# acg-team/ProGraphMSA

Hardware: AMD Instinct MI355X
Metric: DP cell-updates/sec (GCUPS) + wall-clock on 256 seqs × 1000 aa, WAG (higher is better)
Workload: dtype f32

## Files before the change

include/pgm_hip.h:

```cpp
#ifndef PGM_HIP_H_
#define PGM_HIP_H_

#include <stdint.h>
#include <stddef.h>

#ifdef __cplusplus
extern "C" {
#endif

#define PGM_OK 0
#define PGM_ERR_INVALID 1
#define PGM_ERR_DEVICE 2
#define PGM_ERR_BACKTRACK 3
#define PGM_ERR_NOMEM 4

#define PGM_GAP 0xFFFFFFFFu


typedef struct pgm_graph {
    uint32_t n;
    uint32_t dim;
    const double *sites;
    const int32_t *e_rowptr;
    const uint32_t *e_col;
// ... 23 lines not shown
} pgm_align_out;

typedef struct pgm_ctx pgm_ctx;
typedef struct pgm_align_batch pgm_align_batch;

int pgm_device_count(void);
int pgm_ctx_create(int device, pgm_ctx **out);
void pgm_ctx_destroy(pgm_ctx *ctx);
const char *pgm_last_error(void);
int pgm_ctx_device_info(pgm_ctx *ctx, char *name, size_t name_len, int *cu_count);

int pgm_align_graphs_batch(pgm_ctx *ctx, uint32_t njobs, const pgm_graph *const *g1,
                           const pgm_graph *const *g2, const pgm_model *const *model,
                           const pgm_scores *scores, pgm_align_out *out);

int pgm_align_batch_create(pgm_ctx *ctx, uint32_t njobs, const pgm_graph *const *g1,
                           const pgm_graph *const *g2, const pgm_model *const *model,
                           const pgm_scores *scores, pgm_align_batch **out);
#define PGM_BATCH_KEEP_MATRICES 1u
int pgm_align_batch_create_ex(pgm_ctx *ctx, uint32_t njobs, const pgm_graph *const *g1,
                              const pgm_graph *const *g2, const pgm_model *const *model,
                              const pgm_scores *scores, uint32_t flags, pgm_align_batch **out);
typedef struct pgm_site_ref {
    const double *dev_sites;
    const uint32_t *node_map;
    uint32_t ncols;
} pgm_site_ref;
int pgm_align_batch_create_res(pgm_ctx *ctx, uint32_t njobs, const pgm_graph *const *g1,
                               const pgm_graph *const *g2, const pgm_model *const *model,
                               const pgm_scores *scores, uint32_t flags, const pgm_site_ref *res1,
                               const pgm_site_ref *res2, pgm_align_batch **out);
int pgm_align_graphs_batch_res(pgm_ctx *ctx, uint32_t njobs, const pgm_graph *const *g1,
                               const pgm_graph *const *g2, const pgm_model *const *model,
                               const pgm_scores *scores, const pgm_site_ref *res1,
                               const pgm_site_ref *res2, pgm_align_out *out);
int pgm_align_batch_run(pgm_ctx *ctx, pgm_align_batch *b);
int pgm_align_batch_fetch(pgm_ctx *ctx, pgm_align_batch *b, pgm_align_out *out);
void pgm_align_batch_destroy(pgm_ctx *ctx, pgm_align_batch *b);
uint64_t pgm_align_batch_cells(const pgm_align_batch *b);
int pgm_align_batch_time(pgm_ctx *ctx, pgm_align_batch *b, int reps, float *ms_prep,
                         float *ms_emission, float *ms_fill, float *ms_traceback);
int pgm_align_batch_stage_times(pgm_align_batch *b, int reset, float *ms_prep, float *ms_emission, float *ms_fill,
                                uint32_t *launches);
int pgm_align_batch_job_times(pgm_ctx *ctx, pgm_align_batch *b, uint64_t *ticks);
int pgm_align_batch_test_stall(pgm_align_batch *b, uint32_t job, uint32_t band, uint32_t spin_limit);
int pgm_test_cu_shares(uint32_t cus, double lean_cost, uint32_t nlean, double band_cost, uint32_t nbands, double rest_cost,
                       uint32_t nrest, uint32_t ncrit, double longest_chain, uint32_t *out4);
#define PGM_PLAN_HEAD 23
#define PGM_PLAN_DHEAD 9
#define PGM_PLAN_JOB 19
int pgm_test_batch_plan(uint32_t njobs, const pgm_graph *const *g1, const pgm_graph *const *g2, const pgm_model *const *model,
                        const pgm_scores *scores, uint32_t flags, const pgm_site_ref *res1, const pgm_site_ref *res2, uint32_t cus,
                        uint32_t *head, double *dhead, uint32_t *job_fields, uint32_t *items, uint32_t *bands, uint32_t *lean_list, int32_t *tblist);
int pgm_align_batch_read_matrices(pgm_ctx *ctx, pgm_align_batch *b, uint32_t job, float *M,
                                  float *X, float *Y, float *W, float *S);

int pgm_nw_pairs_batch(pgm_ctx *ctx, uint32_t dim, const int32_t *score, int32_t gap_open,
                       int32_t gap_extend, uint32_t nseq, const int8_t *syms,
                       const uint32_t *offs, uint32_t npairs, const uint32_t *pi,
                       const uint32_t *pj, int32_t *counts, uint32_t *gaps);
#define PGM_NW_REDUCED 1u
int pgm_nw_pairs_submit(pgm_ctx *ctx, uint32_t dim, const int32_t *score, int32_t gap_open,
                        int32_t gap_extend, uint32_t nseq, const int8_t *syms,
                        const uint32_t *offs, uint32_t npairs, const uint32_t *pi,
                        const uint32_t *pj, uint32_t flags, int32_t *counts, uint32_t *gaps, int *ticket);
int pgm_nw_pairs_wait(pgm_ctx *ctx, int ticket);
float pgm_nw_last_kernel_ms(pgm_ctx *ctx);
void *pgm_host_alloc(size_t bytes);
void pgm_host_free(void *p);

int pgm_csprofile_load(pgm_ctx *ctx, uint32_t K, uint32_t ncols, const double *lprofiles,
                       const double *centre, const double *priors);
int pgm_csprofile_create_batch(pgm_ctx *ctx, uint32_t nseq, const int8_t *syms,
                               const uint32_t *offs, const double *tau, const double *pi,
                               const double *p_uniform, double *out, const uint64_t *out_offs);
int pgm_csprofile_create_batch_res(pgm_ctx *ctx, uint32_t nseq, const int8_t *syms,
                                   const uint32_t *offs, const double *tau, const double *pi,
                                   const double *p_uniform, const double **dev);
float pgm_csprofile_last_kernel_ms(pgm_ctx *ctx);

typedef struct pgm_mldist_model {
    uint32_t dim;
    const double *Q, *V, *Vi, *sigma;
    double dist_max, var_max, var_min, cutoff_dist, min_dist, max_dist, indel_rate;
    int32_t mldist, mldist_gap;
} pgm_mldist_model;
int pgm_mldist_batch(pgm_ctx *ctx, const pgm_mldist_model *model, uint32_t npairs, const int32_t *counts,
                     const uint32_t *gaps, const double *seqlen, double *dist, double *var);

int pgm_prealigned_counts_batch(pgm_ctx *ctx, uint32_t dim, uint32_t nrows, uint32_t ncols, const int8_t *rows,
                                uint32_t npairs, const uint32_t *pi, const uint32_t *pj, int32_t *counts,
                                uint32_t *gaps);
int pgm_kmer_cosine(pgm_ctx *ctx, uint32_t nseq, uint32_t ncols, const int32_t *counts, double *cosine);
int pgm_kmer_cosine_multi(pgm_ctx *ctx, uint32_t nfam, const uint32_t *nseq, uint32_t ncols, const int32_t *counts, double *cosine);
int pgm_prealigned_counts_multi(pgm_ctx *ctx, uint32_t dim, uint32_t nfam, const uint32_t *nrows, const uint32_t *ncols,
                                const int8_t *rows, uint32_t npairs, const uint32_t *fam, const uint32_t *pi, const uint32_t *pj,
                                int32_t *counts, uint32_t *gaps);
int pgm_prealigned_counts_resampled(pgm_ctx *ctx, uint32_t dim, uint32_t nrows, uint32_t ncols, const int8_t *rows, uint32_t nrep,
                                    const uint32_t *cols, uint32_t npairs, const uint32_t *pi, const uint32_t *pj, int32_t *counts,
                                    uint32_t *gaps);
float pgm_dist_last_kernel_ms(pgm_ctx *ctx);

typedef struct pgm_merge_job {
    uint32_t dim, n1, n2, nnodes;
    const double *sites1, *sites2;
    const double *P1, *P2;
// ... 129 lines not shown
```

prographmsa_amd/__init__.py:

```python
import ctypes as C
import os

_HERE = os.path.dirname(os.path.abspath(__file__))
LIB_PATH = os.path.join(_HERE, "lib", "libpgm_hip.so")
PGMSA_PATH = os.path.join(_HERE, "bin", "pgmsa")

PGM_OK, PGM_ERR_INVALID, PGM_ERR_DEVICE, PGM_ERR_BACKTRACK, PGM_ERR_NOMEM = 0, 1, 2, 3, 4
PGM_GAP = 0xFFFFFFFF
PGM_BATCH_KEEP_MATRICES = 1
PGM_NW_REDUCED = 1
PGM_MERGE_RESIDENT = 1


class pgm_graph(C.Structure):
    _fields_ = [("n", C.c_uint32), ("dim", C.c_uint32), ("sites", C.POINTER(C.c_double)),
                ("e_rowptr", C.POINTER(C.c_int32)), ("e_col", C.POINTER(C.c_uint32)), ("e_val", C.POINTER(C.c_float)),
                ("r_rowptr", C.POINTER(C.c_int32)), ("r_col", C.POINTER(C.c_uint32)), ("r_units", C.POINTER(C.c_uint32))]


class pgm_model(C.Structure):
    _fields_ = [("M", C.POINTER(C.c_double)), ("pi", C.POINTER(C.c_double))]


class pgm_scores(C.Structure):
    _fields_ = [(n, C.c_float) for n in ("gap_init", "gap_extend", "match_init", "end_match", "end_gap", "end_skip",
                                         "start_gap", "start_init", "repeat_init", "repeat_ext")]


class pgm_mldist_model(C.Structure):
    _fields_ = [("dim", C.c_uint32), ("Q", C.POINTER(C.c_double)), ("V", C.POINTER(C.c_double)), ("Vi", C.POINTER(C.c_double)),
                ("sigma", C.POINTER(C.c_double))] + [(n, C.c_double) for n in ("dist_max", "var_max", "var_min", "cutoff_dist", "min_dist", "max_dist", "indel_rate")] \
        + [("mldist", C.c_int32), ("mldist_gap", C.c_int32)]


class pgm_merge_job(C.Structure):
    _fields_ = [("dim", C.c_uint32), ("n1", C.c_uint32), ("n2", C.c_uint32), ("nnodes", C.c_uint32),
                ("sites1", C.POINTER(C.c_double)), ("sites2", C.POINTER(C.c_double)), ("P1", C.POINTER(C.c_double)), ("P2", C.POINTER(C.c_double)),
                ("k1", C.POINTER(C.c_uint32)), ("k2", C.POINTER(C.c_uint32)), ("g2_with_P1", C.POINTER(C.c_uint8)), ("profiles", C.POINTER(C.c_double))]


class pgm_site_ref(C.Structure):
    _fields_ = [("dev_sites", C.POINTER(C.c_double)), ("node_map", C.POINTER(C.c_uint32)), ("ncols", C.c_uint32)]


class pgm_gapmask_job(C.Structure):
    _fields_ = [("src", C.POINTER(C.c_uint64)), ("mapping", C.POINTER(C.c_uint32)), ("dst", C.POINTER(C.c_uint64)),
                ("nrows", C.c_uint32), ("ncols_in", C.c_uint32), ("ncols_out", C.c_uint32)]


class pgm_parsimony_job(C.Structure):
    _fields_ = [("masks", C.POINTER(C.c_uint64)), ("children", C.POINTER(C.c_uint32)), ("nleaves", C.c_uint32), ("ncols", C.c_uint32)]


class pgm_wls_job(C.Structure):
    _fields_ = [("label", C.POINTER(C.c_int8)), ("offset", C.POINTER(C.c_double)), ("nsub", C.c_uint32)]


class pgm_bionj_join(C.Structure):
    _fields_ = [("index1", C.c_uint32), ("index2", C.c_uint32), ("dist1", C.c_double), ("dist2", C.c_double)]


class pgm_bionj_pair(C.Structure):
    _fields_ = [("index1", C.c_uint32), ("index2", C.c_uint32)]


class pgm_align_out(C.Structure):
    _fields_ = [("score", C.c_float), ("n_tr_indels", C.c_uint32), ("len", C.c_uint32), ("status", C.c_int32),
                ("map1", C.POINTER(C.c_uint32)), ("map2", C.POINTER(C.c_uint32))]


EXPORTS = [
    "pgm_device_count", "pgm_ctx_create", "pgm_ctx_destroy", "pgm_last_error", "pgm_ctx_device_info",
    "pgm_align_graphs_batch", "pgm_align_batch_create", "pgm_align_batch_create_ex", "pgm_align_batch_create_res", "pgm_align_graphs_batch_res", "pgm_align_batch_run", "pgm_align_batch_fetch",
    "pgm_align_batch_destroy", "pgm_align_batch_cells", "pgm_align_batch_test_stall", "pgm_test_cu_shares", "pgm_test_batch_plan", "pgm_align_batch_stage_times", "pgm_align_batch_job_times", "pgm_align_batch_time", "pgm_align_batch_read_matrices",
    "pgm_nw_pairs_batch", "pgm_nw_pairs_submit", "pgm_nw_pairs_wait", "pgm_nw_last_kernel_ms", "pgm_host_alloc", "pgm_host_free", "pgm_csprofile_load", "pgm_csprofile_create_batch", "pgm_csprofile_create_batch_res",
    "pgm_csprofile_last_kernel_ms", "pgm_mldist_batch", "pgm_prealigned_counts_batch", "pgm_kmer_cosine", "pgm_dist_last_kernel_ms",
    "pgm_kmer_cosine_multi", "pgm_prealigned_counts_multi", "pgm_prealigned_counts_resampled",
    "pgm_merge_profiles_batch", "pgm_merge_profiles_batch_ex", "pgm_resident_reset", "pgm_resident_onehot", "pgm_resident_import", "pgm_merge_last_kernel_ms",
    "pgm_gapmask_extend_batch", "pgm_gap_parsimony_batch", "pgm_parsimony_last_kernel_ms",
    "pgm_wls_load", "pgm_wls_pair_sums_batch", "pgm_wls_last_kernel_ms", "pgm_wls_last_launches",
    "pgm_bionj", "pgm_bionj_multi", "pgm_bionj_last_launches", "pgm_bionj_last_kernel_ms",
    "pgm_bionj_plan", "pgm_bionj_plan_multi",
    "pgm_msa_agreement", "pgm_agreement_last_kernel_ms",
    "pgm_transfer_min", "pgm_transfer_last_kernel_ms", "pgm_transfer_taxa",
    "pgm_tree_likelihood", "pgm_treelik_last_kernel_ms", "pgm_tree_likelihood_rates", "pgm_tree_ancestral", "pgm_tree_nni", "pgm_tree_nni_edge", "pgm_tree_spr",
    "pgm_tree_ancestral_joint", "pgm_tree_ancestral_sample",
    "pgm_resampled_sums", "pgm_resample_last_kernel_ms",
]


def _load():
    if not os.path.exists(LIB_PATH):
        raise ImportError("libpgm_hip.so is not built (%s); run `python -c 'import __graft_entry__ as g; g.build()'` "
                          "— there is no CPU fallback for the hot path" % LIB_PATH)
    lib = C.CDLL(LIB_PATH)
    vp, u32, i32 = C.c_void_p, C.c_uint32, C.c_int32
    PG, PM = C.POINTER(C.POINTER(pgm_graph)), C.POINTER(C.POINTER(pgm_model))
    sig = {
        "pgm_device_count": (C.c_int, []),
        "pgm_ctx_create": (C.c_int, [C.c_int, C.POINTER(vp)]),
        "pgm_ctx_destroy": (None, [vp]),
        "pgm_last_error": (C.c_char_p, []),
        "pgm_ctx_device_info": (C.c_int, [vp, C.c_char_p, C.c_size_t, C.POINTER(C.c_int)]),
        "pgm_align_graphs_batch": (C.c_int, [vp, u32, PG, PG, PM, C.POINTER(pgm_scores), C.POINTER(pgm_align_out)]),
        "pgm_align_batch_create": (C.c_int, [vp, u32, PG, PG, PM, C.POINTER(pgm_scores), C.POINTER(vp)]),
        "pgm_align_batch_create_ex": (C.c_int, [vp, u32, PG, PG, PM, C.POINTER(pgm_scores), u32, C.POINTER(vp)]),
        "pgm_align_batch_create_res": (C.c_int, [vp, u32, PG, PG, PM, C.POINTER(pgm_scores), u32, C.POINTER(pgm_site_ref), C.POINTER(pgm_site_ref), C.POINTER(vp)]),
        "pgm_align_graphs_batch_res": (C.c_int, [vp, u32, PG, PG, PM, C.POINTER(pgm_scores), C.POINTER(pgm_site_ref), C.POINTER(pgm_site_ref), C.POINTER(pgm_align_out)]),
        "pgm_align_batch_run": (C.c_int, [vp, vp]),
        "pgm_align_batch_fetch": (C.c_int, [vp, vp, C.POINTER(pgm_align_out)]),
        "pgm_align_batch_destroy": (None, [vp, vp]),
        "pgm_align_batch_cells": (C.c_uint64, [vp]),
        "pgm_align_batch_test_stall": (C.c_int, [vp, u32, u32, u32]),
        "pgm_test_cu_shares": (C.c_int, [u32, C.c_double, u32, C.c_double, u32, C.c_double, u32, u32, C.c_double, C.POINTER(C.c_uint32)]),
        "pgm_test_batch_plan": (C.c_int, [u32, PG, PG, PM, C.POINTER(pgm_scores), u32, C.POINTER(pgm_site_ref), C.POINTER(pgm_site_ref), u32,
                                          C.POINTER(u32), C.POINTER(C.c_double)] + [C.POINTER(u32)] * 4 + [C.POINTER(i32)]),
        "pgm_align_batch_stage_times": (C.c_int, [vp, C.c_int] + [C.POINTER(C.c_float)] * 3 + [C.POINTER(u32)]),
        "pgm_align_batch_job_times": (C.c_int, [vp, vp, C.POINTER(C.c_uint64)]),
        "pgm_align_batch_time": (C.c_int, [vp, vp, C.c_int] + [C.POINTER(C.c_float)] * 4),
        "pgm_align_batch_read_matrices": (C.c_int, [vp, vp, u32] + [C.POINTER(C.c_float)] * 5),
        "pgm_nw_pairs_batch": (C.c_int, [vp, u32, C.POINTER(i32), i32, i32, u32, C.POINTER(C.c_int8), C.POINTER(u32), u32,
                                         C.POINTER(u32), C.POINTER(u32), C.POINTER(i32), C.POINTER(u32)]),
        "pgm_nw_pairs_submit": (C.c_int, [vp, u32, C.POINTER(i32), i32, i32, u32, C.POINTER(C.c_int8), C.POINTER(u32), u32,
                                          C.POINTER(u32), C.POINTER(u32), u32, C.POINTER(i32), C.POINTER(u32), C.POINTER(C.c_int)]),
        "pgm_nw_pairs_wait": (C.c_int, [vp, C.c_int]),
        "pgm_host_alloc": (vp, [C.c_size_t]),
        "pgm_host_free": (None, [vp]),
        "pgm_nw_last_kernel_ms": (C.c_float, [vp]),
        "pgm_csprofile_load": (C.c_int, [vp, u32, u32] + [C.POINTER(C.c_double)] * 3),
        "pgm_csprofile_create_batch": (C.c_int, [vp, u32, C.POINTER(C.c_int8), C.POINTER(u32)] + [C.POINTER(C.c_double)] * 4
                                       + [C.POINTER(C.c_uint64)]),
        "pgm_csprofile_create_batch_res": (C.c_int, [vp, u32, C.POINTER(C.c_int8), C.POINTER(u32)] + [C.POINTER(C.c_double)] * 3
                                           + [C.POINTER(C.POINTER(C.c_double))]),
        "pgm_csprofile_last_kernel_ms": (C.c_float, [vp]),
        "pgm_mldist_batch": (C.c_int, [vp, C.POINTER(pgm_mldist_model), u32, C.POINTER(i32), C.POINTER(u32)] + [C.POINTER(C.c_double)] * 3),
        "pgm_prealigned_counts_batch": (C.c_int, [vp, u32, u32, u32, C.POINTER(C.c_int8), u32, C.POINTER(u32), C.POINTER(u32), C.POINTER(i32), C.POINTER(u32)]),
        "pgm_kmer_cosine": (C.c_int, [vp, u32, u32, C.POINTER(i32), C.POINTER(C.c_double)]),
        "pgm_dist_last_kernel_ms": (C.c_float, [vp]),
        "pgm_kmer_cosine_multi": (C.c_int, [vp, u32, C.POINTER(u32), u32, C.POINTER(i32), C.POINTER(C.c_double)]),
        "pgm_prealigned_counts_multi": (C.c_int, [vp, u32, u32, C.POINTER(u32), C.POINTER(u32), C.POINTER(C.c_int8), u32, C.POINTER(u32), C.POINTER(u32),
                                                  C.POINTER(u32), C.POINTER(i32), C.POINTER(u32)]),
        "pgm_prealigned_counts_resampled": (C.c_int, [vp, u32, u32, u32, C.POINTER(C.c_int8), u32, C.POINTER(u32), u32, C.POINTER(u32), C.POINTER(u32),
                                                      C.POINTER(i32), C.POINTER(u32)]),
        "pgm_merge_profiles_batch": (C.c_int, [vp, u32, C.POINTER(pgm_merge_job)]),
        "pgm_merge_profiles_batch_ex": (C.c_int, [vp, u32, C.POINTER(pgm_merge_job), u32, C.POINTER(C.POINTER(C.c_double))]),
        "pgm_resident_reset": (C.c_int, [vp]),
        "pgm_resident_onehot": (C.c_int, [vp, u32, u32, C.POINTER(C.c_int8), C.POINTER(u32), C.POINTER(C.POINTER(C.c_double))]),
        "pgm_resident_import": (C.c_int, [vp, vp, C.POINTER(C.c_double), C.c_uint64, C.POINTER(C.POINTER(C.c_double))]),
        "pgm_merge_last_kernel_ms": (C.c_float, [vp]),
        "pgm_gapmask_extend_batch": (C.c_int, [vp, u32, C.POINTER(pgm_gapmask_job)]),
        "pgm_gap_parsimony_batch": (C.c_int, [vp, u32, C.POINTER(pgm_parsimony_job), C.POINTER(u32)]),
        "pgm_parsimony_last_kernel_ms": (C.c_float, [vp]),
        "pgm_wls_load": (C.c_int, [vp, u32, C.POINTER(C.c_double), C.POINTER(C.c_double)]),
        "pgm_wls_pair_sums_batch": (C.c_int, [vp, u32, C.POINTER(pgm_wls_job), C.POINTER(C.c_double)]),
        "pgm_wls_last_kernel_ms": (C.c_float, [vp]),
        "pgm_wls_last_launches": (C.c_uint32, [vp]),
        "pgm_bionj": (C.c_int, [vp, u32, C.POINTER(C.c_double), C.POINTER(C.c_double), C.POINTER(pgm_bionj_join), C.POINTER(C.c_double)]),
        "pgm_bionj_multi": (C.c_int, [vp, u32, C.POINTER(u32), C.POINTER(C.c_double), C.POINTER(C.c_double), C.POINTER(pgm_bionj_join), C.POINTER(C.c_double)]),
        "pgm_bionj_last_launches": (C.c_uint32, [vp]),
        "pgm_bionj_last_kernel_ms": (C.c_float, [vp]),
        "pgm_bionj_plan": (C.c_int, [vp, u32, C.POINTER(C.c_double), C.POINTER(C.c_double), C.POINTER(pgm_bionj_pair), C.POINTER(pgm_bionj_join), C.POINTER(C.c_double)]),
        "pgm_bionj_plan_multi": (C.c_int, [vp, u32, C.POINTER(u32), C.POINTER(C.c_double), C.POINTER(C.c_double), C.POINTER(pgm_bionj_pair), C.POINTER(pgm_bionj_join), C.POINTER(C.c_double)]),
        "pgm_msa_agreement": (C.c_int, [vp, u32, u32, u32, C.POINTER(i32), C.POINTER(u32), C.POINTER(u32)]),
        "pgm_agreement_last_kernel_ms": (C.c_float, [vp]),
        "pgm_transfer_min": (C.c_int, [vp, u32, u32, C.POINTER(C.c_uint64), u32, C.POINTER(u32), C.POINTER(C.c_uint64), C.POINTER(u32)]),
        "pgm_transfer_last_kernel_ms": (C.c_float, [vp]),
        "pgm_transfer_taxa": (C.c_int, [vp, u32, u32, C.POINTER(C.c_uint64), C.POINTER(u32), u32, C.POINTER(u32), C.POINTER(C.c_uint64),
                                        C.POINTER(u32), C.POINTER(u32), C.POINTER(u32), C.POINTER(u32)]),
        "pgm_tree_likelihood": (C.c_int, [vp, u32, u32, u32, C.POINTER(u32), u32, C.POINTER(C.c_int8), C.POINTER(C.c_double), C.POINTER(C.c_double), C.c_int,
                                          C.POINTER(C.c_double), C.POINTER(i32), C.POINTER(C.c_double), C.POINTER(C.c_double)]),
        "pgm_treelik_last_kernel_ms": (C.c_float, [vp]),
        "pgm_tree_likelihood_rates": (C.c_int, [vp, u32, u32, u32, C.POINTER(u32), u32, C.POINTER(C.c_int8), C.POINTER(C.c_double), u32, C.POINTER(C.c_double),
                                                C.POINTER(C.c_double), C.c_int, C.POINTER(C.c_double), C.POINTER(i32), C.POINTER(C.c_double), C.POINTER(C.c_double),
# ... 317 lines not shown
```

prographmsa_amd/csrc/pgm_align_kernels.h:

```cpp
#ifndef PGM_ALIGN_KERNELS_H_
#define PGM_ALIGN_KERNELS_H_

#include <hip/hip_runtime.h>
#include <math.h>
#include <type_traits>
#include "pgm_device.h"

#define PGM_NEG_INF (-INFINITY)

__device__ __forceinline__ float pgm_ls_log_add(float x, float add) {
    const float a = 2.44247459618085927548717403238913328776812604856113966238617812902399112761292613763080658235564f;
    const float b = -4.2040783745848554315883301529007786406310628696382695994938550046831869207082846248658671f;
    const float c = -0.72123729809042963774358701619456664388406302428056983119308906451199556380646306f;
    const uint32_t bits = __float_as_uint(x);
    const float e = (float)((int32_t)(bits >> 23) - 126);
    const float d = __uint_as_float(((bits << 9) >> 9) ^ 0x3f000000u);
    float t = __fdiv_rn(b, __fsub_rn(d, c));
    const float u = __fadd_rn(e, a);
    t = __fadd_rn(t, add);
    t = __fadd_rn(t, u);
    return t;
}

__device__ __forceinline__ float pgm_emission_finish(float num, float ay, float bx, float match_init) {
    float q = __fdiv_rn(num, __fmul_rn(ay, bx));
    if (q != q) q = __uint_as_float(0xFFC00000u);
    return pgm_ls_log_add(q, match_init);
}

template <int DMAX, int NODES>
__global__ void __launch_bounds__(NODES) pgm_prep_kernel(const PgmJob *__restrict__ jobs, int *__restrict__ sync, uint32_t sync_ints) {
    extern __shared__ float prep_lds[];
    {
        const uint32_t nthreads = gridDim.x * gridDim.y * gridDim.z * NODES;
        const uint32_t gid = ((blockIdx.z * gridDim.y + blockIdx.y) * gridDim.x + blockIdx.x) * NODES + threadIdx.x;
        for (uint32_t i = gid; i < sync_ints; i += nthreads) sync[i] = 0;
    }
    const PgmJob &J = jobs[blockIdx.x];
    const bool first = blockIdx.y == 0;
    const uint32_t n = first ? J.n1 : J.n2;
    const uint32_t v0 = blockIdx.z * NODES;
    if (v0 >= n) return;
    if (J.tabhdr && J.tabhdr[0] == 0) {
        const uint32_t nc = J.dim + 2u;
        bool any = n - 1u >= v0 && n - 1u < v0 + (uint32_t)NODES;
        for (uint32_t c = 0; c < nc; ++c) {
            const uint32_t r = (uint32_t)J.tabhdr[1u + (first ? 0u : nc) + c];
            any = any || (r != 0u && r - 1u >= v0 && r - 1u < v0 + (uint32_t)NODES);
        }
        if (!any) return;
    }
    const uint32_t D = J.dim, DP = J.dp, ST = D + 1;
    float *Mf = prep_lds;
    float *pif = prep_lds + D * D;
    float *nl = pif + D;
    const uint32_t nn = min((uint32_t)NODES, n - v0);
    {
        const int32_t *pp = first ? J.pp1 : J.pp2;
        const uint32_t *pc = first ? J.pc1 : J.pc2, *pu = first ? J.pu1 : J.pu2;
        const float *pv = first ? J.pv1 : J.pv2;
        PgmTbNode *rec = (first ? J.tb1 : J.tb2) + v0;
        for (uint32_t i = threadIdx.x; i < nn * PGM_TB_PK; i += NODES) {
            const uint32_t node = i / PGM_TB_PK, k = i % PGM_TB_PK;
            const int32_t eb = pp[v0 + node];
            const uint32_t cnt = (uint32_t)(pp[v0 + node + 1] - eb);
            const int32_t e = cnt == 0u ? 0 : eb + (int32_t)min(k, cnt - 1u);
            if (k == 0) rec[node].cnt = cnt;
            rec[node].c[k] = pc[e]; rec[node].v[k] = pv[e]; rec[node].u[k] = pu[e];
        }
    }
    if (!first) for (uint32_t i = threadIdx.x; i < D * D; i += NODES) Mf[i] = (float)J.M[i];
    for (uint32_t i = threadIdx.x; i < D; i += NODES) pif[i] = (float)J.pi[i];
    const double *sites = first ? J.sites1 : J.sites2;
    const uint32_t *smap = first ? J.smap1 : J.smap2;
    float *dst = (first ? J.g1f : J.t2) + (size_t)DP * v0;
    for (uint32_t i = threadIdx.x; i < nn * D; i += NODES) {
        const uint32_t node = v0 + i / D;
        const float g = (float)sites[(size_t)D * (smap ? smap[node] : node) + i % D];
        nl[(i / D) * ST + (i % D)] = g;
        if (first && DP == D) dst[i] = g;
// ... 44 lines not shown
        const uint32_t node = i / DP, k = i % DP;
        dst[i] = k < D ? nl[node * ST + k] : 0.0f;
    }
}

#define PGM_TAB_HDR 136
__global__ void __launch_bounds__(256) pgm_classify_kernel(const PgmJob *__restrict__ jobs) {
    const PgmJob &J = jobs[blockIdx.x];
    if (!J.tabhdr) return;
    const bool first = blockIdx.y == 0;
    const uint32_t n = first ? J.n1 : J.n2, D = J.dim;
    const double *sites = first ? J.sites1 : J.sites2;
    const uint32_t *smap = first ? J.smap1 : J.smap2;
    uint8_t *cls = (uint8_t *)(first ? J.cls1 : J.cls2);
    const float uni = (float)(1.0 / (double)D);
    for (uint32_t v = blockIdx.z * blockDim.x + threadIdx.x; v < n; v += gridDim.z * blockDim.x) {
        const double *col = sites + (size_t)D * (smap ? smap[v] : v);
        uint32_t nz = 0, sym = 0;
        bool same = true;
        float vs = 0.f;
        const float g0 = (float)col[0];
        for (uint32_t k = 0; k < D; ++k) {
            const float g = (float)col[k];
            if (g != 0.0f) { ++nz; sym = k; vs = g; }
            same = same && g == g0;
        }
        uint32_t c = 255u;
        if (nz == 0u) c = D + 1u;
        else if (nz == 1u && vs == 1.0f) c = sym;
        else if (same && g0 == uni) c = D;
        cls[v] = (uint8_t)c;
        if (c == 255u) atomicOr(J.tabhdr, 1);
        else atomicCAS(J.tabhdr + 1 + (first ? 0u : D + 2u) + c, 0, (int)v + 1);
    }
}

__device__ __forceinline__ size_t pgm_cell_index(const PgmJob &J, uint32_t y, uint32_t x) {
    const uint32_t b = y / PGM_ROWS, l = PGM_HALO + (y - b * PGM_ROWS);
    return ((size_t)b * J.tsteps + (x + l)) * 64u + l;
}
__device__ __forceinline__ float4 pgm_load_cell(const PgmJob &J, uint32_t y, uint32_t x) {
    return J.cells[pgm_cell_index(J, y, x)];
}

__device__ __forceinline__ float pgm_dpp_wave_shr1(float src, float lane0_value) {
    return __int_as_float(__builtin_amdgcn_update_dpp(__float_as_int(lane0_value), __float_as_int(src), 0x138, 0xf, 0xf, false));
}

#define PGM_GLOBAL __attribute__((address_space(1)))
typedef float pgm_v4f __attribute__((ext_vector_type(4)));
template <class T> __device__ __forceinline__ T pgm_gld(const T *p) { return *(const PGM_GLOBAL T *)(uintptr_t)p; }
#define PGM_EM_TB 4
template <int DP, int RB>
__global__ void __launch_bounds__(4 * PGM_ROWS) pgm_emission_skew_kernel(const PgmJob *__restrict__ jobs) {
    typedef float pgm_v2f __attribute__((ext_vector_type(2)));
    constexpr int NT = DP / 4;
    constexpr int COLS = 64 + PGM_EM_TB * PGM_BLOCK - PGM_HALO - 1;
    constexpr int STR = DP + 1;
    __shared__ pgm_v2f tp[(COLS + 1) * STR];
    __shared__ float bq[COLS];
    const PgmJob &J = jobs[blockIdx.z];
    const uint32_t tb0 = blockIdx.x * PGM_EM_TB;
    const uint32_t rsh = J.rshift, nvb = J.nb << rsh;
    if (tb0 >= J.nblk || 4u * RB * blockIdx.y >= nvb) return;
    if (J.tabhdr && pgm_gld(J.tabhdr) == 0) return;
    auto row_of = [&](uint32_t v, uint32_t lane_) { return ((((v >> rsh) << 6) + lane_) << rsh) | (v & ((1u << rsh) - 1u)); };
    auto sblock_of = [&](uint32_t v, uint32_t tb_) { return ((((size_t)(v >> rsh) * J.nblk + tb_) << rsh) | (v & ((1u << rsh) - 1u))); };
    const uint32_t t0 = tb0 * PGM_BLOCK;
    const int cbase = (int)t0 - 63;
    if ((DP == 20 || DP == 4) && RB == 1) {
        constexpr int TE = DP + 1;
        float *const tab = (float *)tp;
        static_assert(COLS * TE <= (COLS + 1) * STR * 2, "score table must fit the column staging area");
        static_assert(DP > 20 || TE <= 32, "row classes must fit As");
        __shared__ float As[32];
        const uint32_t fb0 = 4u * blockIdx.y + threadIdx.x / PGM_ROWS;
        const uint32_t fl = threadIdx.x % PGM_ROWS;
        const bool active = fb0 < nvb;
        int sym = DP;
        bool plain = true;
        float a_row = 0.f;
        if (active) {
            const uint32_t y = row_of(fb0, fl);
            const uint32_t yc = (y + 1 < J.n1) ? y : 0u;
            const float4 *src = (const float4 *)(J.g1f + (size_t)DP * yc);
            int nz = 0;
#pragma unroll
            for (int q = 0; q < NT; ++q) {
                const float4 v = src[q];
                const float vv[4] = {v.x, v.y, v.z, v.w};
#pragma unroll
                for (int u = 0; u < 4; ++u)
                    if (vv[u] != 0.0f) { ++nz; sym = 4 * q + u; plain = plain && vv[u] == 1.0f; }
            }
            plain = plain && nz <= 1;
            a_row = J.a1[yc];
        }
        if (threadIdx.x < 32) As[threadIdx.x] = 0.f;
        if (__syncthreads_and(plain ? 1 : 0)) {
            if (active) As[sym] = a_row;
            __syncthreads();
            const float mi = J.sc.match_init;
            constexpr int NE = (COLS * TE + 4 * PGM_ROWS - 1) / (4 * PGM_ROWS);
            float tt[NE], tb2[NE];
#pragma unroll
            for (int e = 0; e < NE; ++e) {
                const int i = (int)threadIdx.x + e * 4 * PGM_ROWS;
// ... 17 lines not shown
                if (tb >= J.nblk) break;
                float out[PGM_BLOCK];
#pragma unroll
                for (int i = 0; i < PGM_BLOCK; ++i) out[i] = tab[((int)(tb * PGM_BLOCK) + i - l - cbase) * TE + sym];
                PGM_GLOBAL pgm_v4f *dst = Sq + (sblock_of(fb0, tb) * 64u + (uint32_t)l) * (PGM_BLOCK / 4);
#pragma unroll
                for (int q = 0; q < PGM_BLOCK / 4; ++q) dst[q] = pgm_v4f{out[4 * q], out[4 * q + 1], out[4 * q + 2], out[4 * q + 3]};
            }
            return;
        }
    }
    const float4 *t2q = (const float4 *)J.t2;
    float *tpf = (float *)tp;
    for (int i = threadIdx.x; i < (COLS + 1) * NT; i += 4 * PGM_ROWS) {
        const int ci = i / NT, q = i % NT, c = cbase + ci;
        float4 v = make_float4(0.f, 0.f, 0.f, 0.f);
        if (c >= 0 && c <= (int)J.ncol) v = t2q[(size_t)NT * c + q];
        const float vv[4] = {v.x, v.y, v.z, v.w};
#pragma unroll
        for (int u = 0; u < 4; ++u) {
            const int k = 4 * q + u;
            if (ci < COLS) tpf[2 * (ci * STR + k)] = vv[u];
            if (ci > 0) tpf[2 * ((ci - 1) * STR + k) + 1] = vv[u];
        }
    }
    for (int i = threadIdx.x; i < COLS; i += 4 * PGM_ROWS) {
        const int col = cbase + i;
        bq[i] = (col >= 0 && col <= (int)J.ncol) ? J.b2[col] : 0.f;
    }
    __syncthreads();
    const uint32_t b0 = (4u * blockIdx.y + threadIdx.x / PGM_ROWS) * RB;
    const int l = PGM_HALO + (int)(threadIdx.x % PGM_ROWS);
    if (b0 >= nvb) return;
    float gy[RB][DP], ay[RB];
#pragma unroll
    for (int r = 0; r < RB; ++r) {
        const uint32_t y = row_of(b0 + (uint32_t)r, (uint32_t)(l - PGM_HALO));
        const uint32_t yc = (y + 1 < J.n1) ? y : 0u;
        const float4 *src = (const float4 *)(J.g1f + (size_t)DP * yc);
#pragma unroll
        for (int q = 0; q < NT; ++q) {
            const float4 v = src[q];
            gy[r][4 * q] = v.x; gy[r][4 * q + 1] = v.y; gy[r][4 * q + 2] = v.z; gy[r][4 * q + 3] = v.w;
        }
        ay[r] = J.a1[yc];
    }
    const float mi = J.sc.match_init;
    const uint32_t nblk = J.nblk;
    PGM_GLOBAL pgm_v4f *const Sq = (PGM_GLOBAL pgm_v4f *)(uintptr_t)J.S;
#pragma unroll 1
    for (int w = 0; w < PGM_EM_TB; ++w) {
        const uint32_t tb = tb0 + w;
        if (tb >= nblk) break;
        float out[RB][PGM_BLOCK];
#pragma unroll
        for (int i = 0; i < PGM_BLOCK; i += 2) {
            const int ci = (int)(tb * PGM_BLOCK) + i - l - cbase;
            const pgm_v2f *tc = tp + ci * STR;
            pgm_v2f acc[RB];
#pragma unroll
            for (int r = 0; r < RB; ++r) acc[r] = pgm_v2f{0.0f, 0.0f};
#pragma unroll
            for (int k = 0; k < DP; ++k) {
                const pgm_v2f tk = tc[k];
#pragma unroll
                for (int r = 0; r < RB; ++r) {
                    const pgm_v2f g = {gy[r][k], gy[r][k]};
                    acc[r] = acc[r] + g * tk;
                }
            }
#pragma unroll
            for (int r = 0; r < RB; ++r) {
                out[r][i] = pgm_emission_finish(acc[r].x, ay[r], bq[ci], mi);
                out[r][i + 1] = pgm_emission_finish(acc[r].y, ay[r], bq[ci + 1], mi);
            }
        }
#pragma unroll
        for (int r = 0; r < RB; ++r) {
            if (b0 + (uint32_t)r < nvb) {
                PGM_GLOBAL pgm_v4f *dst = Sq + (sblock_of(b0 + (uint32_t)r, tb) * 64u + (uint32_t)l) * (PGM_BLOCK / 4);
#pragma unroll
                for (int q = 0; q < PGM_BLOCK / 4; ++q) dst[q] = pgm_v4f{out[r][4 * q], out[r][4 * q + 1], out[r][4 * q + 2], out[r][4 * q + 3]};
            }
        }
    }
}

__device__ __forceinline__ int pgm_wave_max8(uint32_t v) {
    int m = __builtin_amdgcn_ballot_w64(v >= 8u) != 0 ? 8 : 0;
    m += __builtin_amdgcn_ballot_w64(v >= (uint32_t)(m + 4)) != 0 ? 4 : 0;
    m += __builtin_amdgcn_ballot_w64(v >= (uint32_t)(m + 2)) != 0 ? 2 : 0;
    m += __builtin_amdgcn_ballot_w64(v >= (uint32_t)(m + 1)) != 0 ? 1 : 0;
    return m;
}

__device__ __forceinline__ __amdgpu_buffer_rsrc_t pgm_band_rsrc(float4 *base, uint32_t bytes) {
    const uint64_t p = (uint64_t)base;
    const uint32_t lo = __builtin_amdgcn_readfirstlane((uint32_t)p), hi = __builtin_amdgcn_readfirstlane((uint32_t)(p >> 32));
    return __builtin_amdgcn_make_buffer_rsrc((void *)(((uint64_t)hi << 32) | lo), 0, __builtin_amdgcn_readfirstlane(bytes), 0x00020000);
}
__device__ __forceinline__ void pgm_store_cell_masked(__amdgpu_buffer_rsrc_t rsrc, uint32_t t, int lane, bool on, float Mv, float Xv, float Wv, float Yv) {
    typedef uint32_t pgm_v4u __attribute__((ext_vector_type(4)));
    pgm_v4u v;
    v.x = __float_as_uint(Mv); v.y = __float_as_uint(Xv); v.z = __float_as_uint(Wv); v.w = __float_as_uint(Yv);
    __builtin_amdgcn_raw_buffer_store_b128(v, rsrc, (on ? (uint32_t)lane * 16u : 0x80000000u) + t * 1024u, 0, 16);
}
__device__ __forceinline__ float4 pgm_gload4(const float4 *p) {
    const pgm_v4f v = *(const PGM_GLOBAL pgm_v4f *)(uintptr_t)p;
    return make_float4(v.x, v.y, v.z, v.w);
}
__device__ __forceinline__ float2 pgm_gload_cell_wy(const float4 *p) {
    const unsigned long long v = __hip_atomic_load((const PGM_GLOBAL unsigned long long *)(uintptr_t)p + 1, __ATOMIC_RELAXED, __HIP_MEMORY_SCOPE_AGENT);
    return make_float2(__uint_as_float((uint32_t)v), __uint_as_float((uint32_t)(v >> 32)));
}
__device__ __forceinline__ float2 pgm_load_cell_mx(const float4 *p) {
    const unsigned long long v = __hip_atomic_load((const PGM_GLOBAL unsigned long long *)(uintptr_t)p, __ATOMIC_RELAXED, __HIP_MEMORY_SCOPE_AGENT);
    return make_float2(__uint_as_float((uint32_t)v), __uint_as_float((uint32_t)(v >> 32)));
}
__device__ __forceinline__ float2 pgm_load_cell_wy(const float4 *p) {
    const unsigned long long v = __hip_atomic_load((const PGM_GLOBAL unsigned long long *)(uintptr_t)p + 1, __ATOMIC_RELAXED, __HIP_MEMORY_SCOPE_AGENT);
    return make_float2(__uint_as_float((uint32_t)v), __uint_as_float((uint32_t)(v >> 32)));
}

struct PgmPred {
    const int32_t *pp; const uint32_t *pc; const float *pv; const uint32_t *pu;
};
__device__ __forceinline__ float pgm_mark_value(const PgmPred &P, int32_t e) {
    const uint32_t u = P.pu[e];
    if (u == 0) return P.pv[e];
    const uint32_t units = u & 0x7fffffffu;
    if (units == 0) return INFINITY;
    return __fadd_rn(INFINITY, __fmul_rn(INFINITY, (float)(units - 1)));
}

struct PgmMapOut {
// ... 2212 lines not shown
```

prographmsa_amd/csrc/pgm_capi.hip:

```cpp
#include <hip/hip_runtime.h>

#include <algorithm>
#include <cmath>
#include <cstdio>
#include <thread>
#include <atomic>
#include <chrono>
#include <queue>
#include <cstdlib>
#include <cstring>
#include <numeric>
#include <optional>
#include <mutex>
#include <string>
#include <unordered_set>
#include <vector>
#include <sys/mman.h>

#include "pgm_align_kernels.h"
#include "pgm_crit_kernels.h"
#include "pgm_nw_kernels.h"
#include "pgm_csprofile_kernels.h"
#include "pgm_dist_kernels.h"
#include "pgm_merge_kernels.h"
// ... 820 lines not shown
        if (res.status != PGM_OK) rc = res.status;
        if (copied[i]) continue;
        out[i].score = res.score;
        out[i].n_tr_indels = res.n_tr_indels;
        out[i].len = res.len;
        out[i].status = res.status;
        if (res.status != PGM_OK) rc = res.status;
        if (!out[i].map1 || !out[i].map2) return fail(PGM_ERR_INVALID, "null mapping buffer");
        if (res.len > b->jobs[i].n1 + b->jobs[i].n2) return fail(PGM_ERR_DEVICE, "corrupt result length");
        memcpy(out[i].map1, b->h_out + b->map1_off[i], 4 * (size_t)res.len);
        memcpy(out[i].map2, b->h_out + b->map2_off[i], 4 * (size_t)res.len);
    }
    if (rc != PGM_OK) g_err = "backtracking failed";
    return rc;
}

void pgm_align_batch_destroy(pgm_ctx *ctx, pgm_align_batch *b) {
    if (!b) return;
    if (ctx) { (void)hipSetDevice(ctx->device); (void)hipStreamSynchronize(ctx->stream); }
    if (ctx && ctx->stream2) (void)hipStreamSynchronize(ctx->stream2);
    if (ctx && ctx->stream3) (void)hipStreamSynchronize(ctx->stream3);
    if (ctx && ctx->stream4) (void)hipStreamSynchronize(ctx->stream4);
    for (int k = 0; k < 5; ++k)
        if (b->ev[k]) (void)hipEventDestroy(b->ev[k]);
    if (b->ev_fork) (void)hipEventDestroy(b->ev_fork);
    if (b->ev_join) (void)hipEventDestroy(b->ev_join);
    if (b->ev_join_b) (void)hipEventDestroy(b->ev_join_b);
    if (b->ev_join_c) (void)hipEventDestroy(b->ev_join_c);
    for (const BatchBuffer &e : kBatchBuffers) cache_give(ctx, e.slot, b->*e.ptr, b->cap[e.slot]);
    cache_give(ctx, pgm_ctx::C_HOST, b->h_out, b->cap[pgm_ctx::C_HOST]);
    cache_give(ctx, pgm_ctx::C_HIN, b->h_in, b->cap[pgm_ctx::C_HIN]);
    delete b;
}

uint64_t pgm_align_batch_cells(const pgm_align_batch *b) { return b ? b->cells : 0; }

int pgm_align_batch_stage_times(pgm_align_batch *b, int reset, float *ms_prep, float *ms_emission, float *ms_fill, uint32_t *launches) {
    if (!b) return fail(PGM_ERR_INVALID, "null batch");
    const double n = b->acc_n ? (double)b->acc_n : 1.0;
    if (ms_prep) *ms_prep = (float)(b->acc_ms[0] / n);
    if (ms_emission) *ms_emission = (float)(b->acc_ms[1] / n);
    if (ms_fill) *ms_fill = (float)(b->acc_ms[2] / n);
    if (launches) *launches = b->acc_n;
    if (reset) { b->acc_ms[0] = b->acc_ms[1] = b->acc_ms[2] = 0; b->acc_n = 0; }
    return PGM_OK;
}

int pgm_align_batch_test_stall(pgm_align_batch *b, uint32_t job, uint32_t band, uint32_t spin_limit) {
    if (!b) return fail(PGM_ERR_INVALID, "null batch");
    b->test_stall_job = job; b->test_stall_band = band; b->test_spin_limit = spin_limit;
    return PGM_OK;
}

int pgm_align_graphs_batch(pgm_ctx *ctx, uint32_t njobs, const pgm_graph *const *g1, const pgm_graph *const *g2,
                           const pgm_model *const *model, const pgm_scores *scores, pgm_align_out *out) {
    return pgm_align_graphs_batch_res(ctx, njobs, g1, g2, model, scores, nullptr, nullptr, out);
}

int pgm_align_graphs_batch_res(pgm_ctx *ctx, uint32_t njobs, const pgm_graph *const *g1, const pgm_graph *const *g2,
                               const pgm_model *const *model, const pgm_scores *scores, const pgm_site_ref *res1, const pgm_site_ref *res2,
                               pgm_align_out *out) {
    pgm_align_batch *b = nullptr;
    const bool prof = getenv("PGM_HOST_PROFILE") != nullptr;
    const auto t0 = std::chrono::steady_clock::now();
    int rc = pgm_align_batch_create_res(ctx, njobs, g1, g2, model, scores, 0u, res1, res2, &b);
    if (rc != PGM_OK) return rc;
    const auto t1 = std::chrono::steady_clock::now();
    {
        static std::mutex device_turn[64];
        std::lock_guard<std::mutex> turn(device_turn[(unsigned)ctx->device % 64u]);
        rc = pgm_align_batch_run(ctx, b);
        if (rc == PGM_OK) rc = pgm_align_batch_fetch(ctx, b, out);
    }
    const auto t2 = std::chrono::steady_clock::now();
    pgm_align_batch_destroy(ctx, b);
    if (prof)
        fprintf(stderr, "  pgm_align_graphs_batch: %u jobs, create (flatten, allocate, upload, work list) %.2f ms, run + fetch %.2f ms, destroy %.2f ms\n", njobs,
                std::chrono::duration<double, std::milli>(t1 - t0).count(), std::chrono::duration<double, std::milli>(t2 - t1).count(),
                std::chrono::duration<double, std::milli>(std::chrono::steady_clock::now() - t2).count());
    return rc;
}

int pgm_align_batch_read_matrices(pgm_ctx *ctx, pgm_align_batch *b, uint32_t job, float *M, float *X, float *Y, float *W, float *S) {
    if (!ctx || !b || job >= b->njobs) return fail(PGM_ERR_INVALID, "bad argument");
    HIPCHK(hipSetDevice(ctx->device));
    HIPCHK(hipStreamSynchronize(ctx->stream));
    const PgmJob &J = b->jobs[job];
    const size_t N = (size_t)J.n1 * J.n2;
    if ((M || X || Y || W) && !J.keep_cells)
        return fail(PGM_ERR_INVALID, "the DP matrices of a chain-only job are only kept for a batch created with PGM_BATCH_KEEP_MATRICES");
    if (S && J.tabhdr) {
        int bad = 1;
        HIPCHK(hipMemcpy(&bad, J.tabhdr, sizeof(int), hipMemcpyDeviceToHost));
        if (bad == 0) return fail(PGM_ERR_INVALID, "the score matrix of a job of two sequence graphs is only stored for a batch created with PGM_BATCH_KEEP_MATRICES");
    }
    if (M || X || Y || W) {
        const uint32_t sh = J.rshift, R = 1u << sh;
        const size_t ncell = (size_t)J.nb * J.tsteps * 64u * R;
        std::vector<float4> cells(ncell);
        HIPCHK(hipMemcpy(cells.data(), J.cells, ncell * sizeof(float4), hipMemcpyDeviceToHost));
        float *dst[4] = {M, X, Y, W};
        for (int k = 0; k < 4; ++k)
            if (dst[k]) std::fill(dst[k], dst[k] + N, -INFINITY);
        for (uint32_t y = 0; y + 1 < J.n1; ++y)
            for (uint32_t x = 0; x < J.ncol; ++x) {
                const uint32_t bb = y >> (6u + sh), w = y & ((64u << sh) - 1u), l = w >> sh, r = w & (R - 1u);
// ... 38 lines not shown
```

Baseline: 82.46.

## Vectorize emission finish with fast packed division and wave-uniform range fallback

Replaces the per-element emission finish (IEEE-rounded divide plus log-add) with a packed two-wide path. It uses a reciprocal with Newton refinement for the divide, checks operand exponent ranges across the wave, and falls back to the exact scalar path when any lane is out of range. The emission loop is restructured to compute four columns at a time and store each vector directly instead of buffering the whole block, and waves-per-EU occupancy hints are added. A test entry point checks the bit-exactness of the new path. The risks are extra register pressure, divergence cost when the fallback triggers, and possible rounding differences from the fast division.

```diff
diff --git a/include/pgm_hip.h b/include/pgm_hip.h
--- a/include/pgm_hip.h
+++ b/include/pgm_hip.h
@@ -99,6 +99,8 @@
 int pgm_test_batch_plan(uint32_t njobs, const pgm_graph *const *g1, const pgm_graph *const *g2, const pgm_model *const *model,
                         const pgm_scores *scores, uint32_t flags, const pgm_site_ref *res1, const pgm_site_ref *res2, uint32_t cus,
                         uint32_t *head, double *dhead, uint32_t *job_fields, uint32_t *items, uint32_t *bands, uint32_t *lean_list, int32_t *tblist);
+int pgm_test_emission_finish2(pgm_ctx *ctx, uint32_t mode, uint32_t npairs, const float *num, const float *ay, const float *bx,
+                              float match_init, uint32_t *out_bits, uint64_t *fast_pairs);
 int pgm_align_batch_read_matrices(pgm_ctx *ctx, pgm_align_batch *b, uint32_t job, float *M,
                                   float *X, float *Y, float *W, float *S);
 
diff --git a/prographmsa_amd/__init__.py b/prographmsa_amd/__init__.py
--- a/prographmsa_amd/__init__.py
+++ b/prographmsa_amd/__init__.py
@@ -72,7 +72,7 @@
 EXPORTS = [
     "pgm_device_count", "pgm_ctx_create", "pgm_ctx_destroy", "pgm_last_error", "pgm_ctx_device_info",
     "pgm_align_graphs_batch", "pgm_align_batch_create", "pgm_align_batch_create_ex", "pgm_align_batch_create_res", "pgm_align_graphs_batch_res", "pgm_align_batch_run", "pgm_align_batch_fetch",
-    "pgm_align_batch_destroy", "pgm_align_batch_cells", "pgm_align_batch_test_stall", "pgm_test_cu_shares", "pgm_test_batch_plan", "pgm_align_batch_stage_times", "pgm_align_batch_job_times", "pgm_align_batch_time", "pgm_align_batch_read_matrices",
+    "pgm_align_batch_destroy", "pgm_align_batch_cells", "pgm_align_batch_test_stall", "pgm_test_cu_shares", "pgm_test_batch_plan", "pgm_align_batch_stage_times", "pgm_align_batch_job_times", "pgm_align_batch_time", "pgm_align_batch_read_matrices", "pgm_test_emission_finish2",
     "pgm_nw_pairs_batch", "pgm_nw_pairs_submit", "pgm_nw_pairs_wait", "pgm_nw_last_kernel_ms", "pgm_host_alloc", "pgm_host_free", "pgm_csprofile_load", "pgm_csprofile_create_batch", "pgm_csprofile_create_batch_res",
     "pgm_csprofile_last_kernel_ms", "pgm_mldist_batch", "pgm_prealigned_counts_batch", "pgm_kmer_cosine", "pgm_dist_last_kernel_ms",
     "pgm_kmer_cosine_multi", "pgm_prealigned_counts_multi", "pgm_prealigned_counts_resampled",
@@ -119,6 +119,7 @@
         "pgm_align_batch_job_times": (C.c_int, [vp, vp, C.POINTER(C.c_uint64)]),
         "pgm_align_batch_time": (C.c_int, [vp, vp, C.c_int] + [C.POINTER(C.c_float)] * 4),
         "pgm_align_batch_read_matrices": (C.c_int, [vp, vp, u32] + [C.POINTER(C.c_float)] * 5),
+        "pgm_test_emission_finish2": (C.c_int, [vp, u32, u32] + [C.POINTER(C.c_float)] * 3 + [C.c_float, C.POINTER(u32), C.POINTER(C.c_uint64)]),
         "pgm_nw_pairs_batch": (C.c_int, [vp, u32, C.POINTER(i32), i32, i32, u32, C.POINTER(C.c_int8), C.POINTER(u32), u32,
                                          C.POINTER(u32), C.POINTER(u32), C.POINTER(i32), C.POINTER(u32)]),
         "pgm_nw_pairs_submit": (C.c_int, [vp, u32, C.POINTER(i32), i32, i32, u32, C.POINTER(C.c_int8), C.POINTER(u32), u32,
diff --git a/prographmsa_amd/csrc/pgm_align_kernels.h b/prographmsa_amd/csrc/pgm_align_kernels.h
--- a/prographmsa_amd/csrc/pgm_align_kernels.h
+++ b/prographmsa_amd/csrc/pgm_align_kernels.h
@@ -26,6 +26,85 @@
     float q = __fdiv_rn(num, __fmul_rn(ay, bx));
     if (q != q) q = __uint_as_float(0xFFC00000u);
     return pgm_ls_log_add(q, match_init);
+}
+
+typedef float pgm_f2 __attribute__((ext_vector_type(2)));
+typedef uint32_t pgm_u2 __attribute__((ext_vector_type(2)));
+
+__device__ __forceinline__ pgm_f2 pgm_div2_fast(pgm_f2 n, pgm_f2 d) {
+    const pgm_f2 one = {1.0f, 1.0f};
+    pgm_f2 r = {__builtin_amdgcn_rcpf(d.x), __builtin_amdgcn_rcpf(d.y)};
+    r = __builtin_elementwise_fma(__builtin_elementwise_fma(-d, r, one), r, r);
+    pgm_f2 q = n * r;
+    q = __builtin_elementwise_fma(__builtin_elementwise_fma(-d, q, n), r, q);
+    return __builtin_elementwise_fma(__builtin_elementwise_fma(-d, q, n), r, q);
+}
+
+#define PGM_DIV2_LO 0x30000000u
+#define PGM_DIV2_HI 0x4f7fffffu
+template <int NP>
+__device__ __forceinline__ bool pgm_div2_in_range(const pgm_f2 (&n)[NP], const pgm_f2 (&d)[NP]) {
+    uint32_t hi = 0u, lo = ~0u;
+#pragma unroll
+    for (int p = 0; p < NP; ++p) {
+        const uint32_t n0 = __float_as_uint(n[p].x), n1 = __float_as_uint(n[p].y), d0 = __float_as_uint(d[p].x), d1 = __float_as_uint(d[p].y);
+        hi = max(max(max(max(hi, n0), n1), d0), d1);
+        lo = min(min(min(min(lo, n0), n1), d0), d1);
+    }
+    return hi <= PGM_DIV2_HI && lo >= PGM_DIV2_LO;
+}
+
+__device__ __forceinline__ pgm_f2 pgm_ls_log_add2(pgm_f2 x, float add) {
+    const float a = 2.44247459618085927548717403238913328776812604856113966238617812902399112761292613763080658235564f;
+    const float b = -4.2040783745848554315883301529007786406310628696382695994938550046831869207082846248658671f;
+    const float c = -0.72123729809042963774358701619456664388406302428056983119308906451199556380646306f;
+    const pgm_u2 bits = {__float_as_uint(x.x), __float_as_uint(x.y)};
+    const pgm_f2 e = {(float)((int32_t)(bits.x >> 23) - 126), (float)((int32_t)(bits.y >> 23) - 126)};
+    const pgm_u2 db = ((bits << 9) >> 9) ^ 0x3f000000u;
+    const pgm_f2 d = {__uint_as_float(db.x), __uint_as_float(db.y)};
+    pgm_f2 t = pgm_div2_fast(pgm_f2{b, b}, d - pgm_f2{c, c});
+    const pgm_f2 u = e + pgm_f2{a, a};
+    t = t + pgm_f2{add, add};
+    t = t + u;
+    return t;
+}
+
+template <int NP>
+__device__ __forceinline__ void pgm_emission_finish2(const pgm_f2 (&num)[NP], const pgm_f2 (&ay)[NP], const pgm_f2 (&bx)[NP], float match_init,
+                                                     pgm_f2 (&out)[NP], bool *fast = nullptr) {
+    pgm_f2 den[NP];
+#pragma unroll
+    for (int p = 0; p < NP; ++p) den[p] = ay[p] * bx[p];
+    const bool all_in = __builtin_amdgcn_ballot_w64(!pgm_div2_in_range(num, den)) == 0;
+    if (fast) *fast = all_in;
+    if (all_in) {
+#pragma unroll
+        for (int p = 0; p < NP; ++p) out[p] = pgm_ls_log_add2(pgm_div2_fast(num[p], den[p]), match_init);
+        return;
+    }
+    asm volatile("" ::: "memory");
+#pragma unroll
+    for (int p = 0; p < NP; ++p)
+        out[p] = pgm_f2{pgm_emission_finish(num[p].x, ay[p].x, bx[p].x, match_init), pgm_emission_finish(num[p].y, ay[p].y, bx[p].y, match_init)};
+}
+
+__global__ void __launch_bounds__(256) pgm_test_finish2_kernel(uint32_t mode, uint32_t npairs, const pgm_f2 *__restrict__ num, const pgm_f2 *__restrict__ ay,
+                                                               const pgm_f2 *__restrict__ bx, float mi, pgm_f2 *__restrict__ out,
+                                                               unsigned long long *__restrict__ fast_pairs) {
+    const uint32_t p = blockIdx.x * 256u + threadIdx.x;
+    if (p >= npairs) return;
+    if (mode == 0) {
+        bool fast;
+        const pgm_f2 n[1] = {num[p]}, a[1] = {ay[p]}, b[1] = {bx[p]};
+        pgm_f2 s[1];
+        pgm_emission_finish2(n, a, b, mi, s, &fast);
+        out[p] = s[0];
+        if (fast) atomicAdd(fast_pairs, 1ull);
+    } else if (mode == 1) {
+        out[p] = pgm_div2_fast(num[p], bx[p]);
+    } else {
+        out[p] = pgm_ls_log_add2(num[p], mi);
+    }
 }
 
 template <int DMAX, int NODES>
@@ -176,7 +255,7 @@
 template <class T> __device__ __forceinline__ T pgm_gld(const T *p) { return *(const PGM_GLOBAL T *)(uintptr_t)p; }
 #define PGM_EM_TB 4
 template <int DP, int RB>
-__global__ void __launch_bounds__(4 * PGM_ROWS) pgm_emission_skew_kernel(const PgmJob *__restrict__ jobs) {
+__global__ void __launch_bounds__(4 * PGM_ROWS) __attribute__((amdgpu_waves_per_eu(DP > 20 ? 3 : 7))) pgm_emission_skew_kernel(const PgmJob *__restrict__ jobs) {
     typedef float pgm_v2f __attribute__((ext_vector_type(2)));
     constexpr int NT = DP / 4;
     constexpr int COLS = 64 + PGM_EM_TB * PGM_BLOCK - PGM_HALO - 1;
@@ -300,35 +379,35 @@
     for (int w = 0; w < PGM_EM_TB; ++w) {
         const uint32_t tb = tb0 + w;
         if (tb >= nblk) break;
-        float out[RB][PGM_BLOCK];
-#pragma unroll
-        for (int i = 0; i < PGM_BLOCK; i += 2) {
-            const int ci = (int)(tb * PGM_BLOCK) + i - l - cbase;
-            const pgm_v2f *tc = tp + ci * STR;
-            pgm_v2f acc[RB];
-#pragma unroll
-            for (int r = 0; r < RB; ++r) acc[r] = pgm_v2f{0.0f, 0.0f};
-#pragma unroll
-            for (int k = 0; k < DP; ++k) {
-                const pgm_v2f tk = tc[k];
-#pragma unroll
-                for (int r = 0; r < RB; ++r) {
-                    const pgm_v2f g = {gy[r][k], gy[r][k]};
-                    acc[r] = acc[r] + g * tk;
-                }
-            }
+#pragma unroll
+        for (int q = 0; q < PGM_BLOCK / 4; ++q) {
+            const int ci = (int)(tb * PGM_BLOCK) + 4 * q - l - cbase;
+            pgm_f2 acc[RB][2];
+#pragma unroll
+            for (int h = 0; h < 2; ++h) {
+                const pgm_v2f *tc = tp + (ci + 2 * h) * STR;
+#pragma unroll
+                for (int r = 0; r < RB; ++r) acc[r][h] = pgm_f2{0.0f, 0.0f};
+#pragma unroll
+                for (int k = 0; k < DP; ++k) {
+                    const pgm_v2f tk = tc[k];
+#pragma unroll
+                    for (int r = 0; r < RB; ++r) {
+                        const pgm_v2f g = {gy[r][k], gy[r][k]};
+                        acc[r][h] = acc[r][h] + g * tk;
+                    }
+                }
+            }
+            const pgm_f2 bx[2] = {pgm_f2{bq[ci], bq[ci + 1]}, pgm_f2{bq[ci + 2], bq[ci + 3]}};
 #pragma unroll
             for (int r = 0; r < RB; ++r) {
-                out[r][i] = pgm_emission_finish(acc[r].x, ay[r], bq[ci], mi);
-                out[r][i + 1] = pgm_emission_finish(acc[r].y, ay[r], bq[ci + 1], mi);
-            }
-        }
-#pragma unroll
-        for (int r = 0; r < RB; ++r) {
-            if (b0 + (uint32_t)r < nvb) {
-                PGM_GLOBAL pgm_v4f *dst = Sq + (sblock_of(b0 + (uint32_t)r, tb) * 64u + (uint32_t)l) * (PGM_BLOCK / 4);
-#pragma unroll
-                for (int q = 0; q < PGM_BLOCK / 4; ++q) dst[q] = pgm_v4f{out[r][4 * q], out[r][4 * q + 1], out[r][4 * q + 2], out[r][4 * q + 3]};
+                const pgm_f2 ar[2] = {pgm_f2{ay[r], ay[r]}, pgm_f2{ay[r], ay[r]}};
+                pgm_f2 s[2];
+                pgm_emission_finish2(acc[r], ar, bx, mi, s);
+                if (b0 + (uint32_t)r < nvb) {
+                    PGM_GLOBAL pgm_v4f *dst = Sq + (sblock_of(b0 + (uint32_t)r, tb) * 64u + (uint32_t)l) * (PGM_BLOCK / 4);
+                    dst[q] = pgm_v4f{s[0].x, s[0].y, s[1].x, s[1].y};
+                }
             }
         }
     }
diff --git a/prographmsa_amd/csrc/pgm_capi.hip b/prographmsa_amd/csrc/pgm_capi.hip
--- a/prographmsa_amd/csrc/pgm_capi.hip
+++ b/prographmsa_amd/csrc/pgm_capi.hip
@@ -896,6 +896,34 @@
     return PGM_OK;
 }
 
+int pgm_test_emission_finish2(pgm_ctx *ctx, uint32_t mode, uint32_t npairs, const float *num, const float *ay, const float *bx, float match_init,
+                              uint32_t *out_bits, uint64_t *fast_pairs) {
+    if (!ctx || mode > 2 || !npairs || !num || !out_bits || (mode == 0 && (!ay || !fast_pairs)) || (mode != 2 && !bx))
+        return fail(PGM_ERR_INVALID, "bad argument");
+    HIPCHK(hipSetDevice(ctx->device));
+    const size_t bytes = (size_t)npairs * 2 * sizeof(float);
+    uint8_t *d = nullptr;
+    HIPCHK(hipMalloc((void **)&d, 4 * bytes + sizeof(unsigned long long)));
+    const float *src[3] = {num, mode == 0 ? ay : nullptr, mode != 2 ? bx : nullptr};
+    hipError_t e = hipMemsetAsync(d, 0, 4 * bytes + sizeof(unsigned long long), ctx->stream);
+    for (int k = 0; k < 3 && e == hipSuccess; ++k)
+        if (src[k]) e = hipMemcpyAsync(d + k * bytes, src[k], bytes, hipMemcpyHostToDevice, ctx->stream);
+    if (e == hipSuccess) {
+        hipLaunchKernelGGL(pgm_test_finish2_kernel, dim3((npairs + 255u) / 256u), dim3(256), 0, ctx->stream, mode, npairs, (const pgm_f2 *)d,
+                           (const pgm_f2 *)(d + bytes), (const pgm_f2 *)(d + 2 * bytes), match_init, (pgm_f2 *)(d + 3 * bytes),
+                           (unsigned long long *)(d + 4 * bytes));
+        e = hipGetLastError();
+    }
+    if (e == hipSuccess) e = hipMemcpyAsync(out_bits, d + 3 * bytes, bytes, hipMemcpyDeviceToHost, ctx->stream);
+    unsigned long long nfast = 0;
+    if (e == hipSuccess) e = hipMemcpyAsync(&nfast, d + 4 * bytes, sizeof(nfast), hipMemcpyDeviceToHost, ctx->stream);
+    if (e == hipSuccess) e = hipStreamSynchronize(ctx->stream);
+    (void)hipFree(d);
+    HIPCHK(e);
+    if (fast_pairs) *fast_pairs = nfast;
+    return PGM_OK;
+}
+
 int pgm_align_graphs_batch(pgm_ctx *ctx, uint32_t njobs, const pgm_graph *const *g1, const pgm_graph *const *g2,
                            const pgm_model *const *model, const pgm_scores *scores, pgm_align_out *out) {
     return pgm_align_graphs_batch_res(ctx, njobs, g1, g2, model, scores, nullptr, nullptr, out);
```

Measured after the change: 81.09. -1.7%, worse.
